# malcolmgreaves/deequ

Measured on AMD Instinct MI355X. Metric: rows/sec (whole node) for fused 16-col profile scan; % of HBM peak BW, higher is better.
Workload: dtype f64+int64+utf8; 1 GPU; C5 fused 16-col profile scan (8 f64 + 4 i64 + 4 utf8, 10% nulls) + state merge + incremental StateLoader append; rows_per_gpu=1000000000, chunk_rows=125000000, analyzers=93, parallelism=row-shard x1

## Files before the change

### deequ_amd/csrc/dq_device.h

```cpp
#pragma once

#include <cstdint>

namespace dq {

constexpr int kBlock = 256;
constexpr int kWaves = kBlock / 64;
constexpr int kRowsPerLane = 8;
constexpr int kRowsPerIter = kBlock * kRowsPerLane;
constexpr int kMaxWG = 4096;
constexpr int kTargetWGs = 8192;
constexpr int kMaxCols = 64;
constexpr int kMaxColTasks = 256;
constexpr int kMaxSchemaCols = 1 << 16;
constexpr int kMaxWhere = 8;
constexpr int kHllCopies = 8;
constexpr int kPredAccCopies = 16;
constexpr int kMaxRoots = 32;
constexpr int kMaxCounters = 32;
constexpr int kMaxInstr = 96;
constexpr int kPredStack = 16;
constexpr int kMaxRegexWords = 32768;

enum ColKind : int32_t {
// ... 22 lines not shown
  CV_I16_S = 20, CV_I16_SH = 21, CV_I16_H = 22,
  CV_I8_S = 23, CV_I8_SH = 24, CV_I8_H = 25,
  CV_F32_D = 26, CV_BOOL = 27,
  CV_D128_S = 28, CV_D128_SH = 29, CV_D128_H = 30, CV_D128_D = 31,
};
constexpr int kNumVariants = 32;

struct VariantDesc {
  int32_t variant;
  int32_t kind;
  bool stats, hll, dtype;
  const char* name;
};
inline constexpr VariantDesc kVariants[] = {
    {CV_VALIDITY, CK_NONE, false, false, false, "validity"},
    {CV_F64_S, CK_F64, true, false, false, "f64_stats"},
    {CV_F64_SH, CK_F64, true, true, false, "f64_stats_hll"},
    {CV_F64_H, CK_F64, false, true, false, "f64_hll"},
    {CV_I64_S, CK_I64, true, false, false, "i64_stats"},
    {CV_I64_SH, CK_I64, true, true, false, "i64_stats_hll"},
    {CV_I64_H, CK_I64, false, true, false, "i64_hll"},
    {CV_I32_S, CK_I32, true, false, false, "i32_stats"},
    {CV_I32_SH, CK_I32, true, true, false, "i32_stats_hll"},
    {CV_I32_H, CK_I32, false, true, false, "i32_hll"},
    {CV_UTF8_H, CK_UTF8, false, true, false, "utf8_hll"},
    {CV_LUTF8_H, CK_LUTF8, false, true, false, "large_utf8_hll"},
    {CV_UTF8_D, CK_UTF8, false, false, true, "utf8_dtype"},
    {CV_UTF8_HD, CK_UTF8, false, true, true, "utf8_hll_dtype"},
    {CV_LUTF8_D, CK_LUTF8, false, false, true, "large_utf8_dtype"},
    {CV_LUTF8_HD, CK_LUTF8, false, true, true, "large_utf8_hll_dtype"},
    {CV_F64_D, CK_F64, false, false, true, "f64_dtype"},
    {CV_F32_S, CK_F32, true, false, false, "f32_stats"},
    {CV_F32_SH, CK_F32, true, true, false, "f32_stats_hll"},
    {CV_F32_H, CK_F32, false, true, false, "f32_hll"},
    {CV_I16_S, CK_I16, true, false, false, "i16_stats"},
    {CV_I16_SH, CK_I16, true, true, false, "i16_stats_hll"},
    {CV_I16_H, CK_I16, false, true, false, "i16_hll"},
    {CV_I8_S, CK_I8, true, false, false, "i8_stats"},
    {CV_I8_SH, CK_I8, true, true, false, "i8_stats_hll"},
    {CV_I8_H, CK_I8, false, true, false, "i8_hll"},
    {CV_F32_D, CK_F32, false, false, true, "f32_dtype"},
    {CV_BOOL, CK_BOOL, false, true, false, "bool"},
    {CV_D128_S, CK_D128, true, false, false, "d128_stats"},
    {CV_D128_SH, CK_D128, true, true, false, "d128_stats_hll"},
    {CV_D128_H, CK_D128, false, true, false, "d128_hll"},
    {CV_D128_D, CK_D128, false, false, true, "d128_dtype"},
};
constexpr int32_t cv_kind(int v) { return kVariants[v].kind; }
constexpr bool cv_stats(int v) { return kVariants[v].stats; }
constexpr bool cv_hll(int v) { return kVariants[v].hll; }
constexpr bool cv_dtype(int v) { return kVariants[v].dtype; }
constexpr bool cv_is_str(int v) { return cv_kind(v) == CK_UTF8 || cv_kind(v) == CK_LUTF8; }
constexpr bool cv_is_str_hll(int v) { return cv_is_str(v) && cv_hll(v); }
constexpr int32_t cv_find(int kind, bool stats, bool hll, bool dtype) {
  for (int v = 0; v < (int)(sizeof(kVariants) / sizeof(kVariants[0])); ++v)
    if (kVariants[v].kind == kind && kVariants[v].stats == stats && kVariants[v].hll == hll && kVariants[v].dtype == dtype)
      return v;
  return -1;
}
constexpr bool cv_table_ok() {
  for (int v = 0; v < kNumVariants; ++v)
    if (kVariants[v].variant != v || cv_find(cv_kind(v), cv_stats(v), cv_hll(v), cv_dtype(v)) != v) return false;
  return true;
}
static_assert(sizeof(kVariants) / sizeof(kVariants[0]) == kNumVariants, "one kVariants row per ColVariant");
static_assert(cv_table_ok(), "kVariants: a row out of ColVariant order, or two variants with one description");

constexpr int kMaxFinRanges = 2 * kNumVariants + 1;
struct FinRanges {
  int32_t n;
  int32_t first[kMaxFinRanges], end[kMaxFinRanges], nr[kMaxFinRanges];
};

struct ColTask {
  int32_t variant;
  int32_t col;
  int32_t where;
  int32_t hll_slot;
  int32_t arg;
  int32_t pad[3];
};

struct PairTask {
  int32_t col_x, col_y;
  int32_t kind_x, kind_y;
  int32_t where;
  int32_t pad[3];
};

constexpr int kTileCols = 8;
constexpr int kTilePairs = 32;
struct PairGroup {
  int32_t ncols;
  int32_t npairs;
  int32_t first_pair;
  int32_t where;
  int32_t cols[kTileCols];
  int32_t kinds[kTileCols];
  int8_t pi[kTilePairs], pj[kTilePairs];
};

constexpr int kPairWaves = 2;
constexpr int kPairPos = 8;
constexpr int kPairSlots = 14;
constexpr int kPairMoments = 4;
constexpr int kPairSlotA[kPairSlots] = {0, 2, 4, 6, 0, 2, 4, 6, 0, 2, 4, 6, 0, 2};
// ... 111 lines not shown
```

### deequ_amd/csrc/dq_hash.h

```cpp
#pragma once

#include <cstdint>

#if defined(__HIP__)
#define DQ_HD __host__ __device__ __forceinline__
#else
#define DQ_HD inline
#endif

namespace dq {

DQ_HD uint32_t alignbit32(uint32_t hi, uint32_t lo, uint32_t sh) {
#if defined(__HIP_DEVICE_COMPILE__)
  return __builtin_amdgcn_alignbit(hi, lo, sh);
#else
  return (uint32_t)((((uint64_t)hi << 32) | lo) >> (sh & 31));
#endif
}

constexpr uint64_t XP1 = 0x9E3779B185EBCA87ull;
constexpr uint64_t XP2 = 0xC2B2AE3D27D4EB4Full;
constexpr uint64_t XP3 = 0x165667B19E3779F9ull;
constexpr uint64_t XP4 = 0x85EBCA77C2B2AE63ull;
constexpr uint64_t XP5 = 0x27D4EB2F165667C5ull;
// ... 37 lines not shown
DQ_HD uint64_t mul_c(uint64_t x, uint64_t c) {
#if defined(__HIP_DEVICE_COMPILE__)
  const uint32_t xl = (uint32_t)x, xh = (uint32_t)(x >> 32);
  uint64_t p, carry;
  uint32_t t1, t2;
#define DQ_MUL_BODY                                                                                  \
  ("v_mad_u64_u32 %[p], %[cy], %[xl], %[cl], 0\n\t"                                                  \
   "v_mul_lo_u32 %[t1], %[xl], %[ch]\n\t"                                                             \
   "v_mul_lo_u32 %[t2], %[xh], %[cl]"                                                                \
   : [p] "=&v"(p), [cy] "=&s"(carry), [t1] "=&v"(t1), [t2] "=&v"(t2)                                 \
   : [xl] "v"(xl), [xh] "v"(xh), [cl] "s"((uint32_t)c), [ch] "s"((uint32_t)(c >> 32)))
  if constexpr (VOL) asm volatile DQ_MUL_BODY;
  else asm DQ_MUL_BODY;
#undef DQ_MUL_BODY
  (void)carry;
  const uint32_t hi = (uint32_t)(p >> 32) + t1 + t2;
  return ((uint64_t)hi << 32) | (uint32_t)p;
#else
  return x * c;
#endif
}

template <bool VOL = false>
DQ_HD uint64_t mul32_c(uint32_t x, uint64_t c) {
#if defined(__HIP_DEVICE_COMPILE__)
  uint64_t p, carry;
  uint32_t t;
#define DQ_MUL_BODY                                                                                  \
  ("v_mad_u64_u32 %[p], %[cy], %[x], %[cl], 0\n\t"                                                   \
   "v_mul_lo_u32 %[t], %[x], %[ch]"                                                                  \
   : [p] "=&v"(p), [cy] "=&s"(carry), [t] "=&v"(t)                                                   \
   : [x] "v"(x), [cl] "s"((uint32_t)c), [ch] "s"((uint32_t)(c >> 32)))
  if constexpr (VOL) asm volatile DQ_MUL_BODY;
  else asm DQ_MUL_BODY;
#undef DQ_MUL_BODY
  (void)carry;
  return ((uint64_t)((uint32_t)(p >> 32) + t) << 32) | (uint32_t)p;
#else
  return (uint64_t)x * c;
#endif
}

DQ_HD uint64_t fmix_head(uint64_t h) {
  h ^= h >> 33;
  h = mul_c(h, XP2);
  return h ^ (h >> 29);
}
DQ_HD uint64_t fmix_tail(uint64_t b) {
  const uint64_t h = b * XP3;
  return h ^ (h >> 32);
}
DQ_HD uint64_t fmix64(uint64_t h) { return fmix_tail(fmix_head(h)); }

DQ_HD uint64_t xxh64_long_head(uint64_t v) {
  const uint64_t k = rotl64(mul_c(v, XP2), 31);
  const uint64_t h = mul_c(k, XP1) ^ (kSeed + XP5 + 8);
  return fmix_head(mul_add_c(rotl64(h, 27), XP1, XP4));
}
DQ_HD uint64_t xxh64_int_head(uint32_t v) {
  const uint64_t h = mul32_c(v, XP1) ^ (kSeed + XP5 + 4);
  return fmix_head(mul_add_c(rotl64(h, 23), XP2, XP3));
}
DQ_HD uint64_t xxh64_long(uint64_t v) { return fmix_tail(xxh64_long_head(v)); }
DQ_HD uint64_t xxh64_int(uint32_t v) { return fmix_tail(xxh64_int_head(v)); }

struct MulP5 {
  DQ_HD uint64_t operator()(uint32_t b) const { return (uint64_t)b * XP5; }
};


template <bool VOL = false>
DQ_HD uint64_t xxh64_stripe_round(uint64_t h, uint64_t k1) {
  return mul_add_c<VOL>(rotl64(h ^ mul_c<VOL>(rotl64(mul_c<VOL>(k1, XP2), 31), XP1), 27), XP1, XP4);
}

template <int NR>
DQ_HD uint64_t xxh64_stripes(const uint32_t (&w)[8], uint32_t len, uint64_t& d4p) {
  uint64_t h = kSeed + XP5 + (uint64_t)len;
  const uint32_t nw = len >> 3;
  d4p = ((uint64_t)w[1] << 32) | w[0];
#pragma unroll
  for (uint32_t k = 0; k < (uint32_t)NR; ++k) {
    if (k < nw) {
      h = xxh64_stripe_round<true>(h, ((uint64_t)w[2 * k + 1] << 32) | w[2 * k]);
      d4p = ((uint64_t)w[2 * k + 3] << 32) | w[2 * k + 2];
    }
  }
  return h;
}

template <typename BP>
DQ_HD uint64_t xxh64_tail_head(uint64_t h, uint64_t d4p, uint32_t len, BP bp) {
  const uint32_t d4 = (uint32_t)d4p;
#if defined(__HIP_DEVICE_COMPILE__) && !defined(DQ_JIT)
  const bool has4 = __builtin_amdgcn_inverse_ballot_w64(__builtin_amdgcn_uicmp(len & 4u, 0u, 33 ));
#else
  const bool has4 = (len & 4u) != 0;
#endif
  const uint32_t db = has4 ? (uint32_t)(d4p >> 32) : d4;
  const uint32_t nb = len & 3u;
  uint64_t kb[3];
#pragma unroll
  for (uint32_t j = 0; j < 3; ++j) kb[j] = bp((db >> (8 * j)) & 0xFFu);
  if (has4) h = mul_add_c<true>(rotl64(h ^ mul32_c<true>(d4, XP1), 23), XP2, XP3);
#pragma unroll
  for (uint32_t j = 0; j < 3; ++j)
// ... 62 lines not shown
```

### deequ_amd/csrc/dq_kernels.hip

```cpp
#include <hip/hip_runtime.h>

#include <cstdint>
#include <type_traits>
#include <utility>

#include "dq_device.h"
#include "dq_hash.h"
#include "dq_decimal.h"
#include "dq_lane.h"
#include "dq_shift.h"

namespace dq {

#define DQ_DEC_TABLE static __constant__ const
#include "dq_dec_tables.inc"
#undef DQ_DEC_TABLE
__device__ __forceinline__ DecTab dec_dev_tab() { return DecTab{kDecP10Lo, kDecP10Hi, kDecRcpHi, kDecRcpLo}; }

typedef uint32_t u32x4 __attribute__((ext_vector_type(4)));

__device__ __forceinline__ uint32_t ld32(const uint8_t* base, int64_t a) {
  return *reinterpret_cast<const uint32_t*>(base + a);
}
__device__ __forceinline__ uint32_t read4(const uint8_t* base, int64_t pos) {
// ... 1 lines not shown
  uint32_t sh = (uint32_t)(pos & 3) * 8u;
  uint32_t w0 = ld32(base, a);
  if (sh == 0) return w0;
  uint32_t w1 = ld32(base, a + 4);
  return alignbit32(w1, w0, sh);
}
__device__ __forceinline__ uint64_t read8(const uint8_t* base, int64_t pos) {
  int64_t a = pos & ~int64_t(3);
  uint32_t sh = (uint32_t)(pos & 3) * 8u;
  uint32_t w0 = ld32(base, a), w1 = ld32(base, a + 4);
  if (sh == 0) return ((uint64_t)w1 << 32) | w0;
  uint32_t w2 = ld32(base, a + 8);
  uint32_t lo = alignbit32(w1, w0, sh);
  uint32_t hi = alignbit32(w2, w1, sh);
  return ((uint64_t)hi << 32) | lo;
}

__device__ uint64_t xxh64_bytes(const uint8_t* data, int64_t pos, int64_t n) {
  int64_t off = pos, end = pos + n;
  uint64_t h;
  if (n >= 32) {
    uint64_t v1 = kSeed + XP1 + XP2, v2 = kSeed + XP2, v3 = kSeed, v4 = kSeed - XP1;
    for (; off <= end - 32; off += 32) {
      v1 = rotl64(v1 + read8(data, off) * XP2, 31) * XP1;
      v2 = rotl64(v2 + read8(data, off + 8) * XP2, 31) * XP1;
      v3 = rotl64(v3 + read8(data, off + 16) * XP2, 31) * XP1;
      v4 = rotl64(v4 + read8(data, off + 24) * XP2, 31) * XP1;
    }
    h = rotl64(v1, 1) + rotl64(v2, 7) + rotl64(v3, 12) + rotl64(v4, 18);
    h ^= rotl64(v1 * XP2, 31) * XP1; h = h * XP1 + XP4;
    h ^= rotl64(v2 * XP2, 31) * XP1; h = h * XP1 + XP4;
    h ^= rotl64(v3 * XP2, 31) * XP1; h = h * XP1 + XP4;
    h ^= rotl64(v4 * XP2, 31) * XP1; h = h * XP1 + XP4;
  } else {
    h = kSeed + XP5;
  }
  h += (uint64_t)n;
  for (; off <= end - 8; off += 8) {
    h ^= rotl64(read8(data, off) * XP2, 31) * XP1;
    h = rotl64(h, 27) * XP1 + XP4;
  }
  if (off + 4 <= end) {
    h ^= (uint64_t)read4(data, off) * XP1;
    h = rotl64(h, 23) * XP2 + XP3;
    off += 4;
  }
  for (; off < end; ++off) {
    h ^= (uint64_t)(read4(data, off) & 0xFFu) * XP5;
    h = rotl64(h, 11) * XP1;
  }
  return fmix64(h);
}

__device__ __forceinline__ int32_t hll_q_exact(uint64_t x) {
  return (int32_t)__clzll((long long)((x << 9) | 256ull));
}

__device__ __forceinline__ void hll_update(int32_t* regs, uint64_t x) {
  atomicMax(&regs[(uint32_t)(x >> 55)], hll_q_exact(x));
}

__device__ __forceinline__ void hll_update_if(int32_t* regs, uint64_t x, bool b) {
  atomicMax(&regs[(uint32_t)(x >> 55)], b ? hll_q_exact(x) : -1);
}

__device__ __forceinline__ int32_t ffbh_raw(uint32_t x) {
  int32_t r;
  asm("v_ffbh_u32 %0, %1" : "=v"(r) : "v"(x));
  return r;
}

struct HllKey {
  uint32_t addr;
  int32_t q;
};
__device__ __forceinline__ uint32_t hll_hi_from_fmix(uint64_t b) {
  const uint32_t bl = (uint32_t)b, bh = (uint32_t)(b >> 32);
  return __umulhi(bl, (uint32_t)XP3) + bl * (uint32_t)(XP3 >> 32) + bh * (uint32_t)XP3;
}
__device__ __forceinline__ HllKey hll_key_from_fmix(uint64_t b) {
  const uint32_t hi = hll_hi_from_fmix(b);
  return {(hi >> 21) & 0x7FCu, ffbh_raw(hi << 9)};
}

constexpr int32_t kFloorMin = 13;
__device__ __forceinline__ uint32_t hll_floor_thr(const uint32_t* __restrict__ hll_floor, int32_t slot) {
  if (!hll_floor || slot < 0) return 0u;
  const int32_t qfloor = (int32_t)hll_floor[slot] - 1;
  return qfloor >= kFloorMin ? 1u << (31 - min(qfloor, 22)) : 0u;
}
__device__ __forceinline__ HllKey hll_key_long(uint64_t v) { return hll_key_from_fmix(xxh64_long_head(v)); }
__device__ __forceinline__ HllKey hll_key_int(uint32_t v) { return hll_key_from_fmix(xxh64_int_head(v)); }


struct ColStats {
  double n, mean, m2, sum;
  int64_t isum, count, nan_count;
  double fmin, fmax;
  int64_t pinf, ninf;
  int64_t isum_hi;
};

__device__ __forceinline__ void stats_init(ColStats& s) {
  s.n = 0.0; s.mean = 0.0; s.m2 = 0.0; s.sum = 0.0;
  s.isum = 0; s.count = 0; s.nan_count = 0;
  s.fmin = __longlong_as_double(0x7FF0000000000000ll);
  s.fmax = __longlong_as_double((long long)0xFFF0000000000000ull);
  s.pinf = 0; s.ninf = 0;
  s.isum_hi = 0;
}

__device__ __forceinline__ void stats_merge(ColStats& a, const ColStats& b) {
  double n = a.n + b.n;
  if (b.n != 0.0) {
    if (a.n == 0.0) {
      a.mean = b.mean; a.m2 = b.m2;
    } else {
      double delta = b.mean - a.mean;
      double r = b.n / n;
      a.mean = a.mean + delta * r;
      a.m2 = a.m2 + b.m2 + delta * delta * a.n * r;
    }
  }
  a.n = n;
  a.sum += b.sum;
  {
    const uint64_t lo = (uint64_t)a.isum + (uint64_t)b.isum;
    a.isum_hi = (int64_t)((uint64_t)a.isum_hi + (uint64_t)b.isum_hi + (lo < (uint64_t)a.isum ? 1u : 0u));
    a.isum = (int64_t)lo;
  }
  a.count += b.count;
  a.nan_count += b.nan_count;
  a.fmin = hw_min(a.fmin, b.fmin);
  a.fmax = hw_max(a.fmax, b.fmax);
  a.pinf += b.pinf;
  a.ninf += b.ninf;
}

__device__ __forceinline__ ColStats stats_shfl_xor(const ColStats& s, int m) {
  ColStats o;
  o.n = __shfl_xor(s.n, m); o.mean = __shfl_xor(s.mean, m); o.m2 = __shfl_xor(s.m2, m);
  o.sum = __shfl_xor(s.sum, m);
  o.isum = __shfl_xor(s.isum, m); o.count = __shfl_xor(s.count, m); o.nan_count = __shfl_xor(s.nan_count, m);
  o.fmin = __shfl_xor(s.fmin, m); o.fmax = __shfl_xor(s.fmax, m);
  o.pinf = __shfl_xor(s.pinf, m); o.ninf = __shfl_xor(s.ninf, m);
// ... 93 lines not shown
  if constexpr (KIND == CK_F64) return __builtin_bit_cast(double, ((uint64_t)w2[1] << 32) | w2[0]);
  return __builtin_fma((double)(int32_t)w2[1], 4294967296.0, (double)w2[0]);
}

template <bool INTEGRAL, bool MINMAX_SEP>
__device__ __forceinline__ void masked_moments(LaneMoments& a, double& lo, double& hi, double x, uint64_t b,
                                               double shift, uint64_t ma, uint64_t mb) {
  double d;
  uint64_t save;
  if constexpr (INTEGRAL) {
    asm volatile(
        "s_and_saveexec_b64 %[save], %[ma]\n\t"
        "v_add_f64 %[d], %[x], -%[sh]\n\t"
        "v_lshl_add_u64 %[is], %[b], 0, %[is]\n\t"
        "v_min_f64 %[lo], %[lo], %[x]\n\t"
        "v_max_f64 %[hi], %[hi], %[x]\n\t"
        "v_add_f64 %[sd], %[sd], %[d]\n\t"
        "v_fma_f64 %[sdd], %[d], %[d], %[sdd]\n\t"
        "s_mov_b64 exec, %[save]"
        : [sd] "+v"(a.sd), [sdd] "+v"(a.sdd), [is] "+v"(a.is), [lo] "+v"(lo), [hi] "+v"(hi), [d] "=&v"(d),
          [save] "=&s"(save)
        : [x] "v"(x), [sh] "s"(shift), [b] "v"(b), [ma] "s"(ma)
        : "scc");
  } else if constexpr (!MINMAX_SEP) {
    asm volatile(
        "s_and_saveexec_b64 %[save], %[ma]\n\t"
        "v_add_f64 %[d], %[x], -%[sh]\n\t"
        "v_min_f64 %[lo], %[lo], %[x]\n\t"
        "v_max_f64 %[hi], %[hi], %[x]\n\t"
        "v_add_f64 %[sd], %[sd], %[d]\n\t"
        "v_fma_f64 %[sdd], %[d], %[d], %[sdd]\n\t"
        "s_mov_b64 exec, %[save]"
        : [sd] "+v"(a.sd), [sdd] "+v"(a.sdd), [lo] "+v"(lo), [hi] "+v"(hi), [d] "=&v"(d), [save] "=&s"(save)
        : [x] "v"(x), [sh] "s"(shift), [ma] "s"(ma)
        : "scc");
  } else {
    asm volatile(
        "s_and_saveexec_b64 %[save], %[ma]\n\t"
        "v_add_f64 %[d], %[x], -%[sh]\n\t"
        "v_add_f64 %[sd], %[sd], %[d]\n\t"
        "v_fma_f64 %[sdd], %[d], %[d], %[sdd]\n\t"
        "s_and_b64 exec, %[save], %[mb]\n\t"
        "v_min_f64 %[lo], %[lo], %[x]\n\t"
        "v_max_f64 %[hi], %[hi], %[x]\n\t"
        "s_mov_b64 exec, %[save]"
        : [sd] "+v"(a.sd), [sdd] "+v"(a.sdd), [lo] "+v"(lo), [hi] "+v"(hi), [d] "=&v"(d), [save] "=&s"(save)
        : [x] "v"(x), [sh] "s"(shift), [ma] "s"(ma), [mb] "s"(mb)
        : "scc");
  }
}

template <int KIND, bool STATS, bool HLL, bool FLOOR = false>
__device__ __forceinline__ void numeric_block(const double (&x)[8], const uint64_t (&bits)[8], const uint64_t (&m)[8],
                                              double shift, ColStats& s, LaneMoments& a, int32_t* regs, int32_t& qmin,
                                              uint32_t thr = 0) {
  uint32_t rmin = ~0u;
#pragma unroll
  for (int j = 0; j < 8; ++j) {
    if (STATS) masked_moments<!ck_float(KIND), false>(a, s.fmin, s.fmax, x[j], bits[j], shift, m[j], m[j]);
    if (HLL) {
      if constexpr (FLOOR) {
        const uint64_t b = ck_bytes(KIND) <= 4 ? xxh64_int_head((uint32_t)bits[j]) : xxh64_long_head(bits[j]);
        rmin = min(rmin, hll_hi_from_fmix(b) << 9);
      } else {
        const HllKey key = ck_bytes(KIND) <= 4 ? hll_key_int((uint32_t)bits[j]) : hll_key_long(bits[j]);
        qmin = min(qmin, key.q);
        if (lane_bit(m[j])) atomicMax(reinterpret_cast<int32_t*>(reinterpret_cast<char*>(regs) + key.addr), key.q);
      }
    }
  }
  if (HLL) {
    const bool redo = FLOOR ? rmin < thr : qmin < 0;
    if (__builtin_amdgcn_ballot_w64(redo) != 0) {
#pragma unroll 1
      for (int j = 0; j < 8; ++j) {
        if (lane_bit(m[j])) hll_update(regs, ck_bytes(KIND) <= 4 ? xxh64_int((uint32_t)bits[j]) : xxh64_long(bits[j]));
      }
      qmin = 0;
    }
  }
}

template <int KIND, bool STATS, bool HLL>
__device__ __forceinline__ void float_block_checked(__amdgpu_buffer_rsrc_t vr, const uint32_t* validity,
                                                    const uint32_t* mask, int64_t base, int32_t rem, int32_t vo,
                                                    double shift, ColStats& s, LaneMoments& a, int32_t* regs,
                                                    int64_t& cnt_w, int64_t& nan_v, int64_t& pinf_v, int64_t& ninf_v) {
  constexpr bool kF32 = KIND == CK_F32;
  const int lane = threadIdx.x & 63;
#pragma unroll 1
  for (int j = 0; j < 8; ++j) {
    const int32_t left = rem - 64 * j;
    if (left <= 0) break;
    const uint64_t mj = sel_word(validity, mask, (base + 64 * j) >> 5, left);
    uint64_t b;
    double xv;
    if constexpr (kF32) {
      b = __builtin_amdgcn_raw_buffer_load_b32(vr, vo + j * 256, 0, 2 );
      xv = (double)__builtin_bit_cast(float, (uint32_t)b);
    } else {
      const auto w2 = __builtin_amdgcn_raw_buffer_load_b64(vr, vo + j * 512, 0, 2 );
      b = ((uint64_t)w2[1] << 32) | w2[0];
      xv = __builtin_bit_cast(double, b);
    }
    const uint64_t nf = __builtin_amdgcn_ballot_w64(!__builtin_isfinite(xv)) & mj;
    const uint64_t nanm = __builtin_amdgcn_ballot_w64(xv != xv) & mj;
    const uint64_t inf = nf & ~nanm, pinf = __builtin_amdgcn_ballot_w64(xv > 0.0) & inf;
    if (lane == 0) {
      nan_v += __builtin_popcountll(nanm);
      pinf_v += __builtin_popcountll(pinf);
      ninf_v += __builtin_popcountll(inf & ~pinf);
    }
    if (STATS) {
      const uint64_t mm = mj & ~inf;
      cnt_w += __builtin_popcountll(mm);
      masked_moments<false, true>(a, s.fmin, s.fmax, xv, b, shift, mm, mj & ~nanm);
    } else {
      cnt_w += __builtin_popcountll(mj);
    }
    if (HLL) {
      if (lane_bit(nanm)) b = kF32 ? 0x7FC00000ull : 0x7FF8000000000000ull;
      const HllKey key = kF32 ? hll_key_int((uint32_t)b) : hll_key_long(b);
      if (lane_bit(mj)) {
        if (key.q >= 0) atomicMax(reinterpret_cast<int32_t*>(reinterpret_cast<char*>(regs) + key.addr), key.q);
        else hll_update(regs, kF32 ? xxh64_int((uint32_t)b) : xxh64_long(b));
      }
    }
  }
}

template <int K> struct KindT { using T = double; };
template <> struct KindT<CK_I64> { using T = int64_t; };
template <> struct KindT<CK_I32> { using T = int32_t; };
template <> struct KindT<CK_F32> { using T = float; };
template <> struct KindT<CK_I16> { using T = int16_t; };
template <> struct KindT<CK_I8> { using T = int8_t; };

template <int KIND, bool STATS, bool HLL>
__device__ void numeric_range(const void* values, const uint32_t* validity, const uint32_t* mask,
                              int64_t row0, int64_t row1, ColStats& s, int32_t* regs, uint32_t thr = 0) {
  using T = typename KindT<KIND>::T;
  constexpr bool kLazy = ck_float(KIND) && STATS;
  const int lane = threadIdx.x & 63;
  const int wave = __builtin_amdgcn_readfirstlane(threadIdx.x >> 6);
  const T* v = reinterpret_cast<const T*>(values);
  const __amdgpu_buffer_rsrc_t vr = __builtin_amdgcn_make_buffer_rsrc(
      const_cast<T*>(v + row0), (short)0, (int)((row1 - row0) * (int64_t)sizeof(T)), 0x00020000);
  int64_t nan_v = 0, pinf_v = 0, ninf_v = 0;
  int64_t cnt_w = 0;
  LaneMoments a{0.0, 0.0, 0};
  const double shift =
      STATS ? range_shift(validity, mask, row0, row1, lane, [=](int64_t r) { return range_value<KIND>(vr, r - row0); }) : 0.0;
  int32_t qmin = 0;
  const int32_t nr = (int32_t)(row1 - row0);
  auto block_loop = [&](auto floor_form) __attribute__((always_inline)) {
    constexpr bool FLOOR = decltype(floor_form)::value;
    for (int32_t rb = 0; rb < nr; rb += kRowsPerIter) {
      const int64_t base = row0 + rb + wave * 512;
      const int32_t rem = nr - rb - wave * 512;
      const bool full = rb + kRowsPerIter <= nr;
      uint64_t bits[8], m[8];
      double x[8];
      const int32_t vo = (rb + wave * 512 + lane) * (int32_t)sizeof(T);
#pragma unroll
      for (int j = 0; j < 8; ++j) {
        if constexpr (sizeof(T) == 8) {
          const auto w2 = __builtin_amdgcn_raw_buffer_load_b64(vr, vo + j * 512, 0, 2 );
          bits[j] = ((uint64_t)w2[1] << 32) | w2[0];
          if (KIND == CK_F64) x[j] = __builtin_bit_cast(double, bits[j]);
          else x[j] = __builtin_fma((double)(int32_t)w2[1], 4294967296.0, (double)w2[0]);
        } else if constexpr (KIND == CK_F32) {
          const uint32_t w = __builtin_amdgcn_raw_buffer_load_b32(vr, vo + j * 256, 0, 2 );
          bits[j] = w;
          x[j] = (double)__builtin_bit_cast(float, w);
        } else {
          int32_t w;
          if constexpr (sizeof(T) == 4) w = (int32_t)__builtin_amdgcn_raw_buffer_load_b32(vr, vo + j * 256, 0, 2 );
          else if constexpr (sizeof(T) == 2) w = (int16_t)__builtin_amdgcn_raw_buffer_load_b16(vr, vo + j * 128, 0, 2 );
          else w = (int8_t)__builtin_amdgcn_raw_buffer_load_b8(vr, vo + j * 64, 0, 2 );
          bits[j] = (uint64_t)(int64_t)w;
          x[j] = (double)w;
        }
      }
      block_masks(validity, mask, base, rem, full, m);
      uint64_t nf_any = 0;
      if constexpr (ck_float(KIND) && !kLazy) {
#pragma unroll
        for (int j = 0; j < 8; ++j) nf_any |= __builtin_amdgcn_ballot_w64(!__builtin_isfinite(x[j])) & m[j];
      }
      if (ck_float(KIND) && !kLazy && nf_any != 0) {
        float_block_checked<KIND, STATS, HLL>(vr, validity, mask, base, rem, vo, shift, s, a, regs, cnt_w, nan_v, pinf_v,
                                              ninf_v);
      } else {
#pragma unroll
        for (int j = 0; j < 8; ++j) cnt_w += __builtin_popcountll(m[j]);
        numeric_block<KIND, STATS, HLL, FLOOR>(x, bits, m, shift, s, a, regs, qmin, thr);
      }
    }
  };
  if (HLL && thr != 0) block_loop(std::true_type{});
  else block_loop(std::false_type{});
  if constexpr (kLazy) {
    __shared__ int32_t redo;
    if (threadIdx.x == 0) redo = 0;
    __syncthreads();
    const bool bad = !__builtin_isfinite(a.sd) || !__builtin_isfinite(a.sdd);
    if (__builtin_amdgcn_ballot_w64(bad) != 0 && lane == 0) redo = 1;
    __syncthreads();
    if (redo) {
      if (HLL) {
        for (int i = threadIdx.x; i < 512; i += kBlock) regs[i] = -1;
      }
      stats_init(s);
      a = LaneMoments{0.0, 0.0, 0};
      cnt_w = 0;
      __syncthreads();
      for (int32_t rb = 0; rb < nr; rb += kRowsPerIter) {
        const int32_t vo = (rb + wave * 512 + lane) * (int32_t)sizeof(T);
        float_block_checked<KIND, STATS, HLL>(vr, validity, mask, row0 + rb + wave * 512, nr - rb - wave * 512, vo,
                                              shift, s, a, regs, cnt_w, nan_v, pinf_v, ninf_v);
      }
    }
  }
  if (STATS) {
    const double S1 = wave_sum_f64(a.sd), S2 = wave_sum_f64(a.sdd);
    const int64_t is = ck_float(KIND) ? 0 : wave_sum_i64(a.is);
    if (lane == 0 && cnt_w > 0) {
      const double n = (double)cnt_w, q = S1 / n;
      s.n = n;
      s.mean = shift + q;
      const double m2 = __builtin_fma(-S1, q, S2);
      s.m2 = m2 < 0.0 ? 0.0 : m2;
      if (ck_float(KIND)) s.sum = __builtin_fma(n, shift, S1);
      else s.isum = is;
    }
  }
  if (lane == 0) s.count += cnt_w;
  if (ck_float(KIND) && lane == 0) {
    s.nan_count += nan_v;
    s.pinf += pinf_v;
    s.ninf += ninf_v;
    if (STATS) s.count += pinf_v + ninf_v;
  }
}

enum DtClass : uint32_t { DT_FRACTIONAL = 1, DT_INTEGRAL = 2, DT_BOOLEAN = 3, DT_STRING = 4 };

__device__ __forceinline__ uint32_t dt_class_of(bool numeric, uint32_t dots, bool boolean) {
  return numeric && dots <= 1 ? (dots ? DT_FRACTIONAL : DT_INTEGRAL) : (boolean ? DT_BOOLEAN : DT_STRING);
}

__device__ __forceinline__ uint32_t dt_keep(int lo, int hi) {
  const uint32_t below_hi = hi >= 4 ? 0x80808080u : (hi <= 0 ? 0u : 0x80808080u & ((1u << (8 * hi)) - 1u));
  const uint32_t from_lo = lo <= 0 ? 0x80808080u : (lo >= 4 ? 0u : 0x80808080u & ~((1u << (8 * lo)) - 1u));
  return below_hi & from_lo;
}

__device__ __forceinline__ uint32_t dt_class_short(const uint32_t (&w)[8], uint32_t len, bool active) {
  const uint32_t b0 = w[0] & 0xFFu;
  const uint32_t sgn = (len > 0 && (b0 == 0x2Bu || b0 == 0x2Du)) ? 1u : 0u;
  const uint32_t start = sgn + ((sgn < len && ((w[0] >> (8 * sgn)) & 0xFFu) == 0x20u) ? 1u : 0u);
  uint32_t bad = 0, dots = 0;
#pragma unroll
  for (int k = 0; k < 7; ++k) {
    if (k > 0 && __builtin_amdgcn_ballot_w64(active && bad == 0 && dots <= 1 && (uint32_t)(4 * k) < len) == 0) break;
    const uint32_t keep = dt_keep((int)start - 4 * k, (int)len - 4 * k);
    const uint32_t t = w[k] ^ 0x30303030u, z = w[k] ^ 0x2E2E2E2Eu;
    const uint32_t nd = ((t & 0x7F7F7F7Fu) + 0x76767676u) | t;
    const uint32_t nz = ((z & 0x7F7F7F7Fu) + 0x7F7F7F7Fu) | z;
    bad |= nd & nz & keep;
    dots += __builtin_popcount(~nz & keep);
  }
  const bool boolean = (len == 4 && w[0] == 0x65757274u) ||
// ... 407 lines not shown
      if constexpr (HLL) {
        const uint64_t b = dec_hash_head(lo[j], hi[j], prec);
        const HllKey key = hll_key_from_fmix(b);
        if (sel) {
          if (key.q >= 0) atomicMax(reinterpret_cast<int32_t*>(reinterpret_cast<char*>(regs) + key.addr), key.q);
          else hll_update(regs, fmix_tail(b));
        }
      }
      if constexpr (DT) frac += __builtin_popcountll(__builtin_amdgcn_ballot_w64(dec_dt_class(lo[j], hi[j], sc, tab) == 1) & m[j]);
    }
  }
  if constexpr (STATS) {
    const double S1 = wave_sum_f64(a.sd), S2 = wave_sum_f64(a.sdd), G = wave_sum_f64(guard);
#pragma unroll
    for (int k = 32; k >= 1; k >>= 1) {
      const uint64_t olo = __shfl_xor(slo, k), ohi = __shfl_xor(shi, k);
      const uint64_t l2 = slo + olo;
      shi = shi + ohi + (l2 < slo ? 1u : 0u);
      slo = l2;
    }
    if (lane == 0 && cnt_w > 0) {
      const double n = (double)cnt_w, q = S1 / n;
      s.n = n;
      s.mean = shift + q;
      const double m2 = __builtin_fma(-S1, q, S2);
      s.m2 = m2 < 0.0 ? 0.0 : m2;
      s.sum = G;
      s.isum = (int64_t)slo;
      s.isum_hi = (int64_t)shi;
    }
  }
  if (lane == 0) {
    s.count += cnt_w;
    if (DT) s.isum += frac;
  }
}

__device__ void validity_range(const uint32_t* validity, const uint32_t* mask, int64_t row0, int64_t row1, ColStats& s) {
  const int64_t w0 = row0 >> 5, w1 = (row1 + 31) >> 5;
  int64_t c = 0;
  for (int64_t w = w0 + threadIdx.x; w < w1; w += kBlock) {
    uint32_t bits = word_or_ones(validity, w);
    if (mask) bits &= mask[w];
    const int64_t r = w << 5;
    if (r + 32 > row1) bits &= (1u << (row1 - r)) - 1u;
    c += __popc(bits);
  }
  s.count += c;
}

template <int V, bool LONG>
__device__ __forceinline__ void run_variant(const ColTask& t, const ScanCols& cols, const uint32_t* mask, int64_t row0,
                                            int64_t row1, int64_t n_rows, ColStats& s, int32_t* regs,
                                            const uint64_t* p5, uint32_t* dq, uint32_t* rare, uint32_t thr) {
  const void* v = cols.values[t.col];
  const uint32_t* val = cols.validity[t.col];
  constexpr int K = cv_kind(V);
  constexpr bool S = cv_stats(V), H = cv_hll(V), D = cv_dtype(V);
  if constexpr (K == CK_NONE) validity_range(val, mask, row0, row1, s);
  else if constexpr (ck_float(K) && D)
    float_dtype_range(reinterpret_cast<const typename KindT<K>::T*>(v), val, mask, row0, row1, s);
  else if constexpr (ck_numeric(K)) numeric_range<K, S, H>(v, val, mask, row0, row1, s, regs, thr);
  else if constexpr (K == CK_BOOL) bool_range(reinterpret_cast<const uint32_t*>(v), val, mask, row0, row1, s, regs);
  else if constexpr (K == CK_D128) decimal_range<S, H, D>(v, val, mask, row0, row1, s, regs, t.arg);
  else {
    static_assert(cv_is_str(V), "run_variant: a variant of a kind no case above reads");
    using OffT = std::conditional_t<K == CK_UTF8, int32_t, int64_t>;
    utf8_range<OffT, H, D, LONG>(reinterpret_cast<const uint8_t*>(v), reinterpret_cast<const OffT*>(cols.offsets[t.col]),
                                 val, mask, row0, row1, n_rows, s, regs, p5, dq, rare);
  }
}

#ifndef DQ_STR_WAVES
#define DQ_STR_WAVES 6
#endif
#ifndef DQ_NUM_WAVES
#define DQ_NUM_WAVES 6
#endif
template <int V, bool LONG>
constexpr int kMinWaves = V == CV_UTF8_H && DQ_STR_WAVES > 0 ? DQ_STR_WAVES
                          : (V == CV_F64_SH || V == CV_I64_SH) && DQ_NUM_WAVES > 0 ? DQ_NUM_WAVES
                          : V == CV_LUTF8_H && LONG ? 5
                                                    : 1;

template <int V, bool LONG = false>
__global__ __launch_bounds__(kBlock) __attribute__((amdgpu_waves_per_eu(kMinWaves<V, LONG>))) void dq_column_scan(const ColTask* __restrict__ tasks, int32_t ntasks,
                                                         int32_t part_base, ScanCols cols, ScanBitmaps bm,
                                                         int64_t n_rows, int64_t rows_per_range,
                                                         ColPartial* __restrict__ partials,
                                                         uint32_t* __restrict__ hll_acc,
                                                         const uint32_t* __restrict__ hll_floor) {
  constexpr bool kBool = cv_kind(V) == CK_BOOL;
  constexpr bool kHll = cv_hll(V) && !kBool;
  constexpr bool kStr = cv_is_str_hll(V);
  __shared__ int32_t regs[kHll ? 512 : 2];
  __shared__ uint64_t p5[kStr ? 256 : 1];
  __shared__ uint32_t dfq[kStr ? kWaves * kDefFields * kDefCap : 1];
  __shared__ uint32_t rare[kStr ? kWaves : 1];
  __shared__ ColStats red[kWaves];
  const int32_t ti = blockIdx.x % ntasks;
  const int32_t range = blockIdx.x / ntasks;
  const ColTask t = tasks[ti];
  const int64_t row0 = (int64_t)range * rows_per_range;
  int64_t row1 = row0 + rows_per_range;
  if (row1 > n_rows) row1 = n_rows;
  if constexpr (kBool) {
    if (threadIdx.x < 2) regs[threadIdx.x] = 0;
    __syncthreads();
  }
  if constexpr (kHll) {
    for (int i = threadIdx.x; i < 512; i += kBlock) regs[i] = -1;
    if constexpr (kStr) {
      p5[threadIdx.x] = (uint64_t)threadIdx.x * XP5;
      if (threadIdx.x < kWaves) rare[threadIdx.x] = 0;
    }
    __syncthreads();
  }
  ColStats s;
  stats_init(s);
  const uint32_t* mask = t.where >= 0 ? reinterpret_cast<const uint32_t*>(bm.where_bits[t.where]) : nullptr;
  const int32_t wv = kStr ? __builtin_amdgcn_readfirstlane(threadIdx.x >> 6) : 0;
  run_variant<V, LONG>(t, cols, mask, row0, row1, n_rows, s, regs, p5, dfq + wv * kDefFields * kDefCap, rare + wv,
                       kHll ? hll_floor_thr(hll_floor, t.hll_slot) : 0u);
  block_reduce_store(s, partials + (size_t)(part_base + ti) * kMaxWG + range, red);
  if constexpr (kStr) {
    if (threadIdx.x == 0 && bm.rare_rows) {
      uint32_t r = 0;
      for (int w = 0; w < kWaves; ++w) r += rare[w];
      if (r) atomicAdd(reinterpret_cast<unsigned long long*>(bm.rare_rows + part_base + ti), (unsigned long long)r);
    }
  }
  if constexpr (kBool) {
    if (threadIdx.x == 0 && t.hll_slot >= 0) {
      uint32_t* dst = hll_acc + ((size_t)t.hll_slot * kHllCopies + (blockIdx.x % kHllCopies)) * 512;
      for (int b = 0; b < 2; ++b) {
        if (!regs[b]) continue;
        const uint64_t x = xxh64_int(b == 0 ? 1u : 0u);
        atomicMax(dst + (uint32_t)(x >> 55), (uint32_t)(hll_q_exact(x) + 1));
      }
    }
  }
  if constexpr (kHll) {
    __syncthreads();
    uint32_t* dst = hll_acc + ((size_t)t.hll_slot * kHllCopies + (blockIdx.x % kHllCopies)) * 512;
    for (int i = threadIdx.x; i < 512; i += kBlock) {
      const uint32_t v = (uint32_t)(regs[i] + 1);
      if (v > __builtin_nontemporal_load(dst + i)) atomicMax(dst + i, v);
    }
  }
}

struct CorrStats { double n, xa, ya, ck, xm, ym; };

__device__ __forceinline__ void corr_merge(CorrStats& a, const CorrStats& b) {
  double n = a.n + b.n;
  if (b.n != 0.0) {
    if (a.n == 0.0) { a.xa = b.xa; a.ya = b.ya; a.ck = b.ck; a.xm = b.xm; a.ym = b.ym; }
    else {
      double dx = b.xa - a.xa, dy = b.ya - a.ya;
      double r = b.n / n;
      double dxr = dx * r, dyr = dy * r;
      a.ck = a.ck + b.ck + dx * dyr * a.n;
      a.xm = a.xm + b.xm + dx * dxr * a.n;
      a.ym = a.ym + b.ym + dy * dyr * a.n;
      a.xa = a.xa + dxr;
      a.ya = a.ya + dyr;
    }
  }
  a.n = n;
}

__device__ __forceinline__ int cmp_dbl(double a, double b) {
  bool an = a != a, bn = b != b;
  if (an || bn) return (an && bn) ? 0 : (an ? 1 : -1);
  return (a > b) - (a < b);
}
__device__ __forceinline__ bool apply_cmp(int op, int c) {
  switch (op) {
    case C_LT: return c < 0;
    case C_LE: return c <= 0;
    case C_GT: return c > 0;
    case C_GE: return c >= 0;
    case C_EQ: return c == 0;
    case C_NE: return c != 0;
    case C_TRUE: return true;
    default: return false;
  }
}

struct PredScratch {
  uint32_t *st, *sn, *rt, *rn, *ct, *cn;
  __device__ PredScratch(uint32_t* w, int depth, int roots, int counters) {
    st = w; sn = st + 16 * depth; rt = sn + 16 * depth; rn = rt + 16 * roots; ct = rn + 16 * roots; cn = ct + 16 * counters;
  }
};

__device__ __forceinline__ void pred_load(const void* p, int kind, int64_t row0, int64_t row1, int64_t base, int lane,
                                          uint64_t (&v)[8]) {
  if (kind == CK_BOOL) {
// ... 782 lines not shown
```

Baseline: 29.60 billion rows/s.

## Track HLL registers as minimum shifted hash word for numeric columns

Numeric HLL columns now keep, per register, the minimum of the left-shifted hash word using atomicMin, rather than computing a leading-zero rank per row and applying atomicMax. The rank is derived once per register at flush via clz. Rows whose shifted word is zero, where the rank exceeds the shifted width, fall back to a direct global atomicMax through a shared destination pointer. The goal is to take clz and rank logic out of the per-row hot loop, at the cost of a new register encoding, a rarely taken global-atomic slow path, and extra plumbing of the destination pointer.

Measured after the change: 29.65 billion rows/s, median of 2. About the same (+0.2%).

```diff
diff --git a/deequ_amd/csrc/dq_device.h b/deequ_amd/csrc/dq_device.h
--- a/deequ_amd/csrc/dq_device.h
+++ b/deequ_amd/csrc/dq_device.h
@@ -98,6 +98,7 @@
 constexpr bool cv_dtype(int v) { return kVariants[v].dtype; }
 constexpr bool cv_is_str(int v) { return cv_kind(v) == CK_UTF8 || cv_kind(v) == CK_LUTF8; }
 constexpr bool cv_is_str_hll(int v) { return cv_is_str(v) && cv_hll(v); }
+constexpr bool cv_hll_minw(int v) { return cv_hll(v) && ck_numeric(cv_kind(v)); }
 constexpr int32_t cv_find(int kind, bool stats, bool hll, bool dtype) {
   for (int v = 0; v < (int)(sizeof(kVariants) / sizeof(kVariants[0])); ++v)
     if (kVariants[v].kind == kind && kVariants[v].stats == stats && kVariants[v].hll == hll && kVariants[v].dtype == dtype)
diff --git a/deequ_amd/csrc/dq_hash.h b/deequ_amd/csrc/dq_hash.h
--- a/deequ_amd/csrc/dq_hash.h
+++ b/deequ_amd/csrc/dq_hash.h
@@ -113,6 +113,25 @@
 }
 DQ_HD uint64_t fmix64(uint64_t h) { return fmix_tail(fmix_head(h)); }
 
+#if !defined(DQ_JIT)
+DQ_HD uint32_t mul_c_hi32(uint64_t b, uint64_t c) {
+  const uint32_t bl = (uint32_t)b, bh = (uint32_t)(b >> 32), cl = (uint32_t)c, ch = (uint32_t)(c >> 32);
+#if defined(__HIP_DEVICE_COMPILE__)
+  const uint32_t carry = __umulhi(bl, cl);
+#else
+  const uint32_t carry = (uint32_t)(((uint64_t)bl * cl) >> 32);
+#endif
+  return carry + bl * ch + bh * cl;
+}
+DQ_HD uint32_t hll_hi_from_fmix(uint64_t b) { return mul_c_hi32(b, XP3); }
+DQ_HD int32_t hll_q_exact(uint64_t x) { return (int32_t)__builtin_clzll((x << 9) | 256ull); }
+
+DQ_HD uint32_t hll_minw_pw(uint32_t w_min) {
+  if (w_min == 0xFFFFFFFFu) return 0u;
+  return (w_min ? (uint32_t)__builtin_clz(w_min) : 23u) + 1u;
+}
+#endif
+
 DQ_HD uint64_t xxh64_long_head(uint64_t v) {
   const uint64_t k = rotl64(mul_c(v, XP2), 31);
   const uint64_t h = mul_c(k, XP1) ^ (kSeed + XP5 + 8);
diff --git a/deequ_amd/csrc/dq_kernels.hip b/deequ_amd/csrc/dq_kernels.hip
--- a/deequ_amd/csrc/dq_kernels.hip
+++ b/deequ_amd/csrc/dq_kernels.hip
@@ -77,10 +77,6 @@
   return fmix64(h);
 }
 
-__device__ __forceinline__ int32_t hll_q_exact(uint64_t x) {
-  return (int32_t)__clzll((long long)((x << 9) | 256ull));
-}
-
 __device__ __forceinline__ void hll_update(int32_t* regs, uint64_t x) {
   atomicMax(&regs[(uint32_t)(x >> 55)], hll_q_exact(x));
 }
@@ -99,13 +95,15 @@
   uint32_t addr;
   int32_t q;
 };
-__device__ __forceinline__ uint32_t hll_hi_from_fmix(uint64_t b) {
-  const uint32_t bl = (uint32_t)b, bh = (uint32_t)(b >> 32);
-  return __umulhi(bl, (uint32_t)XP3) + bl * (uint32_t)(XP3 >> 32) + bh * (uint32_t)XP3;
-}
 __device__ __forceinline__ HllKey hll_key_from_fmix(uint64_t b) {
   const uint32_t hi = hll_hi_from_fmix(b);
   return {(hi >> 21) & 0x7FCu, ffbh_raw(hi << 9)};
+}
+
+__device__ __forceinline__ void hll_minw_update(int32_t* regs, uint32_t* const* dst, uint64_t x) {
+  const uint32_t hi = (uint32_t)(x >> 32), w = hi << 9;
+  atomicMin(reinterpret_cast<uint32_t*>(regs) + (hi >> 23), w);
+  if (w == 0) atomicMax(*dst + (hi >> 23), (uint32_t)(hll_q_exact(x) + 1));
 }
 
 constexpr int32_t kFloorMin = 13;
@@ -114,8 +112,6 @@
   const int32_t qfloor = (int32_t)hll_floor[slot] - 1;
   return qfloor >= kFloorMin ? 1u << (31 - min(qfloor, 22)) : 0u;
 }
-__device__ __forceinline__ HllKey hll_key_long(uint64_t v) { return hll_key_from_fmix(xxh64_long_head(v)); }
-__device__ __forceinline__ HllKey hll_key_int(uint32_t v) { return hll_key_from_fmix(xxh64_int_head(v)); }
 
 
 struct ColStats {
@@ -315,31 +311,31 @@
 
 template <int KIND, bool STATS, bool HLL, bool FLOOR = false>
 __device__ __forceinline__ void numeric_block(const double (&x)[8], const uint64_t (&bits)[8], const uint64_t (&m)[8],
-                                              double shift, ColStats& s, LaneMoments& a, int32_t* regs, int32_t& qmin,
-                                              uint32_t thr = 0) {
+                                              double shift, ColStats& s, LaneMoments& a, int32_t* regs,
+                                              uint32_t* const* dst, uint32_t thr = 0) {
   uint32_t rmin = ~0u;
+  uint32_t wprev = 0;
 #pragma unroll
   for (int j = 0; j < 8; ++j) {
     if (STATS) masked_moments<!ck_float(KIND), false>(a, s.fmin, s.fmax, x[j], bits[j], shift, m[j], m[j]);
     if (HLL) {
-      if constexpr (FLOOR) {
-        const uint64_t b = ck_bytes(KIND) <= 4 ? xxh64_int_head((uint32_t)bits[j]) : xxh64_long_head(bits[j]);
-        rmin = min(rmin, hll_hi_from_fmix(b) << 9);
-      } else {
-        const HllKey key = ck_bytes(KIND) <= 4 ? hll_key_int((uint32_t)bits[j]) : hll_key_long(bits[j]);
-        qmin = min(qmin, key.q);
-        if (lane_bit(m[j])) atomicMax(reinterpret_cast<int32_t*>(reinterpret_cast<char*>(regs) + key.addr), key.q);
-      }
+      const uint64_t b = ck_bytes(KIND) <= 4 ? xxh64_int_head((uint32_t)bits[j]) : xxh64_long_head(bits[j]);
+      const uint32_t hi = hll_hi_from_fmix(b), w = hi << 9;
+      if constexpr (!FLOOR) {
+        if (lane_bit(m[j])) atomicMin(reinterpret_cast<uint32_t*>(reinterpret_cast<char*>(regs) + ((hi >> 21) & 0x7FCu)), w);
+      }
+      if (j & 1) rmin = min(min(rmin, wprev), w);
+      else wprev = w;
     }
   }
   if (HLL) {
-    const bool redo = FLOOR ? rmin < thr : qmin < 0;
+    const bool redo = FLOOR ? rmin < thr : rmin == 0;
     if (__builtin_amdgcn_ballot_w64(redo) != 0) {
 #pragma unroll 1
       for (int j = 0; j < 8; ++j) {
-        if (lane_bit(m[j])) hll_update(regs, ck_bytes(KIND) <= 4 ? xxh64_int((uint32_t)bits[j]) : xxh64_long(bits[j]));
-      }
-      qmin = 0;
+        if (lane_bit(m[j]))
+          hll_minw_update(regs, dst, ck_bytes(KIND) <= 4 ? xxh64_int((uint32_t)bits[j]) : xxh64_long(bits[j]));
+      }
     }
   }
 }
@@ -348,7 +344,8 @@
 __device__ __forceinline__ void float_block_checked(__amdgpu_buffer_rsrc_t vr, const uint32_t* validity,
                                                     const uint32_t* mask, int64_t base, int32_t rem, int32_t vo,
                                                     double shift, ColStats& s, LaneMoments& a, int32_t* regs,
-                                                    int64_t& cnt_w, int64_t& nan_v, int64_t& pinf_v, int64_t& ninf_v) {
+                                                    uint32_t* const* dst, int64_t& cnt_w, int64_t& nan_v, int64_t& pinf_v,
+                                                    int64_t& ninf_v) {
   constexpr bool kF32 = KIND == CK_F32;
   const int lane = threadIdx.x & 63;
 #pragma unroll 1
@@ -383,11 +380,7 @@
     }
     if (HLL) {
       if (lane_bit(nanm)) b = kF32 ? 0x7FC00000ull : 0x7FF8000000000000ull;
-      const HllKey key = kF32 ? hll_key_int((uint32_t)b) : hll_key_long(b);
-      if (lane_bit(mj)) {
-        if (key.q >= 0) atomicMax(reinterpret_cast<int32_t*>(reinterpret_cast<char*>(regs) + key.addr), key.q);
-        else hll_update(regs, kF32 ? xxh64_int((uint32_t)b) : xxh64_long(b));
-      }
+      if (lane_bit(mj)) hll_minw_update(regs, dst, kF32 ? xxh64_int((uint32_t)b) : xxh64_long(b));
     }
   }
 }
@@ -401,7 +394,8 @@
 
 template <int KIND, bool STATS, bool HLL>
 __device__ void numeric_range(const void* values, const uint32_t* validity, const uint32_t* mask,
-                              int64_t row0, int64_t row1, ColStats& s, int32_t* regs, uint32_t thr = 0) {
+                              int64_t row0, int64_t row1, ColStats& s, int32_t* regs, uint32_t* const* dst,
+                              uint32_t thr = 0) {
   using T = typename KindT<KIND>::T;
   constexpr bool kLazy = ck_float(KIND) && STATS;
   const int lane = threadIdx.x & 63;
@@ -414,7 +408,6 @@
   LaneMoments a{0.0, 0.0, 0};
   const double shift =
       STATS ? range_shift(validity, mask, row0, row1, lane, [=](int64_t r) { return range_value<KIND>(vr, r - row0); }) : 0.0;
-  int32_t qmin = 0;
   const int32_t nr = (int32_t)(row1 - row0);
   auto block_loop = [&](auto floor_form) __attribute__((always_inline)) {
     constexpr bool FLOOR = decltype(floor_form)::value;
@@ -452,12 +445,12 @@
         for (int j = 0; j < 8; ++j) nf_any |= __builtin_amdgcn_ballot_w64(!__builtin_isfinite(x[j])) & m[j];
       }
       if (ck_float(KIND) && !kLazy && nf_any != 0) {
-        float_block_checked<KIND, STATS, HLL>(vr, validity, mask, base, rem, vo, shift, s, a, regs, cnt_w, nan_v, pinf_v,
-                                              ninf_v);
+        float_block_checked<KIND, STATS, HLL>(vr, validity, mask, base, rem, vo, shift, s, a, regs, dst, cnt_w, nan_v,
+                                              pinf_v, ninf_v);
       } else {
 #pragma unroll
         for (int j = 0; j < 8; ++j) cnt_w += __builtin_popcountll(m[j]);
-        numeric_block<KIND, STATS, HLL, FLOOR>(x, bits, m, shift, s, a, regs, qmin, thr);
+        numeric_block<KIND, STATS, HLL, FLOOR>(x, bits, m, shift, s, a, regs, dst, thr);
       }
     }
   };
@@ -481,7 +474,7 @@
       for (int32_t rb = 0; rb < nr; rb += kRowsPerIter) {
         const int32_t vo = (rb + wave * 512 + lane) * (int32_t)sizeof(T);
         float_block_checked<KIND, STATS, HLL>(vr, validity, mask, row0 + rb + wave * 512, nr - rb - wave * 512, vo,
-                                              shift, s, a, regs, cnt_w, nan_v, pinf_v, ninf_v);
+                                              shift, s, a, regs, dst, cnt_w, nan_v, pinf_v, ninf_v);
       }
     }
   }
@@ -995,7 +988,8 @@
 template <int V, bool LONG>
 __device__ __forceinline__ void run_variant(const ColTask& t, const ScanCols& cols, const uint32_t* mask, int64_t row0,
                                             int64_t row1, int64_t n_rows, ColStats& s, int32_t* regs,
-                                            const uint64_t* p5, uint32_t* dq, uint32_t* rare, uint32_t thr) {
+                                            const uint64_t* p5, uint32_t* dq, uint32_t* rare, uint32_t* const* dst,
+                                            uint32_t thr) {
   const void* v = cols.values[t.col];
   const uint32_t* val = cols.validity[t.col];
   constexpr int K = cv_kind(V);
@@ -1003,7 +997,7 @@
   if constexpr (K == CK_NONE) validity_range(val, mask, row0, row1, s);
   else if constexpr (ck_float(K) && D)
     float_dtype_range(reinterpret_cast<const typename KindT<K>::T*>(v), val, mask, row0, row1, s);
-  else if constexpr (ck_numeric(K)) numeric_range<K, S, H>(v, val, mask, row0, row1, s, regs, thr);
+  else if constexpr (ck_numeric(K)) numeric_range<K, S, H>(v, val, mask, row0, row1, s, regs, dst, thr);
   else if constexpr (K == CK_BOOL) bool_range(reinterpret_cast<const uint32_t*>(v), val, mask, row0, row1, s, regs);
   else if constexpr (K == CK_D128) decimal_range<S, H, D>(v, val, mask, row0, row1, s, regs, t.arg);
   else {
@@ -1037,6 +1031,7 @@
   constexpr bool kHll = cv_hll(V) && !kBool;
   constexpr bool kStr = cv_is_str_hll(V);
   __shared__ int32_t regs[kHll ? 512 : 2];
+  __shared__ uint32_t* hll_dst;
   __shared__ uint64_t p5[kStr ? 256 : 1];
   __shared__ uint32_t dfq[kStr ? kWaves * kDefFields * kDefCap : 1];
   __shared__ uint32_t rare[kStr ? kWaves : 1];
@@ -1053,6 +1048,9 @@
   }
   if constexpr (kHll) {
     for (int i = threadIdx.x; i < 512; i += kBlock) regs[i] = -1;
+    if constexpr (cv_hll_minw(V)) {
+      if (threadIdx.x == 0) hll_dst = hll_acc + ((size_t)t.hll_slot * kHllCopies + (blockIdx.x % kHllCopies)) * 512;
+    }
     if constexpr (kStr) {
       p5[threadIdx.x] = (uint64_t)threadIdx.x * XP5;
       if (threadIdx.x < kWaves) rare[threadIdx.x] = 0;
@@ -1064,7 +1062,7 @@
   const uint32_t* mask = t.where >= 0 ? reinterpret_cast<const uint32_t*>(bm.where_bits[t.where]) : nullptr;
   const int32_t wv = kStr ? __builtin_amdgcn_readfirstlane(threadIdx.x >> 6) : 0;
   run_variant<V, LONG>(t, cols, mask, row0, row1, n_rows, s, regs, p5, dfq + wv * kDefFields * kDefCap, rare + wv,
-                       kHll ? hll_floor_thr(hll_floor, t.hll_slot) : 0u);
+                       &hll_dst, kHll ? hll_floor_thr(hll_floor, t.hll_slot) : 0u);
   block_reduce_store(s, partials + (size_t)(part_base + ti) * kMaxWG + range, red);
   if constexpr (kStr) {
     if (threadIdx.x == 0 && bm.rare_rows) {
@@ -1085,9 +1083,11 @@
   }
   if constexpr (kHll) {
     __syncthreads();
-    uint32_t* dst = hll_acc + ((size_t)t.hll_slot * kHllCopies + (blockIdx.x % kHllCopies)) * 512;
+    uint32_t* dst;
+    if constexpr (cv_hll_minw(V)) dst = hll_dst;
+    else dst = hll_acc + ((size_t)t.hll_slot * kHllCopies + (blockIdx.x % kHllCopies)) * 512;
     for (int i = threadIdx.x; i < 512; i += kBlock) {
-      const uint32_t v = (uint32_t)(regs[i] + 1);
+      const uint32_t v = cv_hll_minw(V) ? hll_minw_pw((uint32_t)regs[i]) : (uint32_t)(regs[i] + 1);
       if (v > __builtin_nontemporal_load(dst + i)) atomicMax(dst + i, v);
     }
   }
```
